# thu-pacman/chitu

Measured on AMD Instinct MI355X. Metric: output tok/s (bs=16) DeepSeek-R1 FP8 TP=8; HBM GB/s vs peak, higher is better.
Workload: dtype fp8_e4m3 weights+activations (W8A8, fp32 accumulate), bf16 attention

## Files before the change

chitu_amd/csrc/fp8_gemm.hip:

```cpp
#include "common.h"
#include "gemm_common.h"
#ifndef CHITU_GEMM_PHASE_MASK
#define CHITU_GEMM_PHASE_MASK 0
#endif

namespace chitu {

typedef long mfma_ab_t;

__device__ __forceinline__ mfma_ab_t pack_lo(const i32x4& v) {
    return (long)(((unsigned long long)(uint32_t)v[1] << 32) | (uint32_t)v[0]);
}
__device__ __forceinline__ mfma_ab_t pack_hi(const i32x4& v) {
    return (long)(((unsigned long long)(uint32_t)v[3] << 32) | (uint32_t)v[2]);
}

template <int MT>
struct GemmStage {
    W8Frag w;
    i32x4 x[MT][2];
    float xs[MT];
    float ws;
};

// ... 41 lines not shown
        const int off = kb << 7;
        if (!(dbg & 8)) {
            st.w.w[0] = __builtin_nontemporal_load(reinterpret_cast<const i32x4*>(wp0 + off));
            st.w.w[1] = __builtin_nontemporal_load(reinterpret_cast<const i32x4*>(wp1 + off));
        } else {
            st.w.w[0] = st.w.w[1] = i32x4{kb, lane, 3, 4};
        }
#pragma unroll
        for (int mt = 0; mt < MT; ++mt) {
            if (TM || (dbg & 16)) {
                st.x[mt][0] = *reinterpret_cast<const i32x4*>(xp[mt] + (size_t)kb * 2048);
                st.x[mt][1] = *reinterpret_cast<const i32x4*>(xp[mt] + (size_t)kb * 2048 + 1024);
            } else if (!(dbg & 1)) {
                st.x[mt][0] = *reinterpret_cast<const i32x4*>(xp[mt] + off);
                st.x[mt][1] = *reinterpret_cast<const i32x4*>(xp[mt] + off + 64);
            } else {
                st.x[mt][0] = st.x[mt][1] = i32x4{kb, lane, 1, 2};
            }
            st.xs[mt] = (dbg & 4) ? 1.0f : (TM || (dbg & 16)) ? xsp[mt][kb * 16] : xsp[mt][kb];
        }
        st.ws = wsp[kb];
    };
    auto compute = [&](const GemmStage<MT>& st) {
#pragma unroll
        for (int mt = 0; mt < MT; ++mt) {
            f32x4 blk;
            if (!(dbg & 2)) blk = w8a8_block_dot(st.w, st.x[mt][0], st.x[mt][1]);
            else
                blk = f32x4{__int_as_float(st.w.w[0][0] ^ st.x[mt][0][0]), __int_as_float(st.w.w[0][1] ^ st.x[mt][1][1]),
                            __int_as_float(st.w.w[1][2] ^ st.x[mt][0][2]), __int_as_float(st.w.w[1][3] ^ st.x[mt][1][3])};
#pragma unroll
            for (int r = 0; r < 4; ++r) acc[mt][r] += (blk[r] * st.xs[mt]) * st.ws;
        }
    };

    constexpr int D = DEEP ? 8 : MT >= 4 ? 2 : 4;
    GemmStage<MT> ring[D];
#pragma unroll
    for (int d = 0; d < D; ++d)
        if (kb0 + d < kb1) load(ring[d], kb0 + d);
    if (DEEP) CHITU_PROBE_MARK(1);
    for (int kb = kb0; kb < kb1; kb += D) {
#pragma unroll
        for (int d = 0; d < D; ++d) {
            if (kb + d < kb1) {
                compute(ring[d]);
                if (DEEP && kb == kb0 && d == 0) {
                    if (acc[0][0] == 1.2345e30f) CHITU_PROBE_MARK(9);
                    CHITU_PROBE_MARK(2);
                }
                if (kb + d + D < kb1) load(ring[d], kb + d + D);
            }
        }
    }
    if (DEEP) {
        if (acc[0][0] == 1.2345e30f) CHITU_PROBE_MARK(9);
        CHITU_PROBE_MARK(3);
    }

    gemm_epilogue_v2<MT, WK>(acc, red, out, out_dt, partial, M, N, S, m_base, n0);
    if (DEEP) CHITU_PROBE_MARK(4);
}

__global__ __launch_bounds__(256) void splitk_reduce_kernel(const float* __restrict__ partial,
                                                            void* __restrict__ out, int out_dt,
                                                            int S, int64_t MN) {
    for (int64_t i = ((int64_t)blockIdx.x * blockDim.x + threadIdx.x) * 4; i < MN;
         i += (int64_t)gridDim.x * blockDim.x * 4) {
        float v[4] = {0.f, 0.f, 0.f, 0.f};
        const int cnt = (int)min((int64_t)4, MN - i);
        for (int s = 0; s < S; ++s)
            for (int r = 0; r < cnt; ++r) v[r] += partial[(size_t)s * MN + i + r];
        for (int r = 0; r < cnt; ++r) {
            if (out_dt == 2) ((float*)out)[i + r] = v[r];
            else ((uint16_t*)out)[i + r] = out_dt == 0 ? f32_to_bf16(v[r]) : f32_to_f16(v[r]);
        }
    }
}

template <int MT, int WK>
__global__ __launch_bounds__(64 * WK) void soft_fp8_gemm_kernel(
    const bf16_t* __restrict__ X, const fp8_t* __restrict__ W, const float* __restrict__ WS,
    void* __restrict__ out, int out_dt, float* __restrict__ partial, int M, int N, int K, int S,
    int m_base) {
// ... 250 lines not shown
```

chitu_amd/csrc/gate.hip:

```cpp
#include "common.h"
#include "gemm_common.h"
#include "moe_align_device.h"

namespace chitu {

template <int MT>
struct Bf16Stage {
    s16x8 w[2];
    s16x8 x[MT][2];
};

template <int MT, int WK, bool DEEP = false>
__global__ __launch_bounds__(64 * WK) void bf16_gemm_kernel(const bf16_t* __restrict__ X,
                                                            const bf16_t* __restrict__ W,
                                                            void* __restrict__ out, int out_dt,
                                                            float* __restrict__ partial, int M, int N,
                                                            int K, int S, int m_base) {
    __shared__ float red[WK > 1 ? WK * MT * 256 : 1];
    const int lane = threadIdx.x & 63, wave = __builtin_amdgcn_readfirstlane(threadIdx.x >> 6);
    const int j = lane & 15, g = lane >> 4;
    const int n0 = blockIdx.x * 16;
    const int KB = K >> 6;
    const int T = S * WK;
    const int t = blockIdx.y * WK + wave;
    const int kb0 = (int)((long)KB * t / T), kb1 = (int)((long)KB * (t + 1) / T);
    const int eoff = ((j & 1) * 4 + g) * 8;
    const bf16_t* wp0 = W + (size_t)min(n0 + (j >> 1), N - 1) * K + eoff;
    const bf16_t* wp1 = W + (size_t)min(n0 + 8 + (j >> 1), N - 1) * K + eoff;
    const bf16_t* xp[MT];
#pragma unroll
    for (int mt = 0; mt < MT; ++mt) xp[mt] = X + (size_t)min(m_base + mt * 16 + j, M - 1) * K + g * 8;
    f32x4 e0[MT], o0[MT], e1[MT], o1[MT];
#pragma unroll
    for (int mt = 0; mt < MT; ++mt) e0[mt] = o0[mt] = e1[mt] = o1[mt] = f32x4{0.f, 0.f, 0.f, 0.f};
    auto load = [&](Bf16Stage<MT>& st, int kb) {
        const int off = kb << 6;
        st.w[0] = __builtin_nontemporal_load(reinterpret_cast<const s16x8*>(wp0 + off));
        st.w[1] = __builtin_nontemporal_load(reinterpret_cast<const s16x8*>(wp1 + off));
#pragma unroll
        for (int mt = 0; mt < MT; ++mt) {
            st.x[mt][0] = *reinterpret_cast<const s16x8*>(xp[mt] + off);
            st.x[mt][1] = *reinterpret_cast<const s16x8*>(xp[mt] + off + 32);
        }
    };
    auto compute = [&](const Bf16Stage<MT>& st) {
#pragma unroll
        for (int mt = 0; mt < MT; ++mt) {
            e0[mt] = __builtin_amdgcn_mfma_f32_16x16x32_bf16(st.w[0], st.x[mt][0], e0[mt], 0, 0, 0);
            o0[mt] = __builtin_amdgcn_mfma_f32_16x16x32_bf16(st.w[0], st.x[mt][1], o0[mt], 0, 0, 0);
            e1[mt] = __builtin_amdgcn_mfma_f32_16x16x32_bf16(st.w[1], st.x[mt][0], e1[mt], 0, 0, 0);
            o1[mt] = __builtin_amdgcn_mfma_f32_16x16x32_bf16(st.w[1], st.x[mt][1], o1[mt], 0, 0, 0);
        }
    };
    constexpr int D = DEEP ? 8 : MT >= 4 ? 2 : 4;
    Bf16Stage<MT> ring[D];
#pragma unroll
    for (int d = 0; d < D; ++d)
        if (kb0 + d < kb1) load(ring[d], kb0 + d);
    for (int kb = kb0; kb < kb1; kb += D) {
#pragma unroll
        for (int d = 0; d < D; ++d) {
            if (kb + d < kb1) {
                compute(ring[d]);
                if (kb + d + D < kb1) load(ring[d], kb + d + D);
            }
        }
    }
    f32x4 acc[MT];
#pragma unroll
    for (int mt = 0; mt < MT; ++mt)
        acc[mt] = f32x4{e0[mt][0] + o0[mt][1], e0[mt][2] + o0[mt][3], e1[mt][0] + o1[mt][1], e1[mt][2] + o1[mt][3]};
    gemm_epilogue_v2<MT, WK>(acc, red, out, out_dt, partial, M, N, S, m_base, n0);
}

template <int MT>
struct Bf16Stage2 {
    s16x8 wg[2], wu[2];
    s16x8 x[MT][2];
};

template <int MT, int WK>
__global__ __launch_bounds__(64 * WK) void bf16_gemm_silu_kernel(const bf16_t* __restrict__ X, const bf16_t* __restrict__ W,
                                                                 bf16_t* __restrict__ out, int M, int inter, int K,
                                                                 int m_base) {
    __shared__ float red[WK > 1 ? WK * MT * 512 : 1];
    const int lane = threadIdx.x & 63, wave = __builtin_amdgcn_readfirstlane(threadIdx.x >> 6);
    const int j = lane & 15, g = lane >> 4;
    const int n0 = blockIdx.x * 16;
    const int KB = K >> 6;
    const int kb0 = KB * wave / WK, kb1 = KB * (wave + 1) / WK;
    const int eoff = ((j & 1) * 4 + g) * 8;
    const int r0 = min(n0 + (j >> 1), inter - 1), r1 = min(n0 + 8 + (j >> 1), inter - 1);
    const bf16_t* gp0 = W + (size_t)r0 * K + eoff;
    const bf16_t* gp1 = W + (size_t)r1 * K + eoff;
    const bf16_t* up0 = W + (size_t)(inter + r0) * K + eoff;
    const bf16_t* up1 = W + (size_t)(inter + r1) * K + eoff;
    const bf16_t* xp[MT];
// ... 841 lines not shown
```

chitu_amd/csrc/gemm_common.h:

```cpp
#pragma once
#include "common.h"

namespace chitu {

template <int MT, int WK>
__device__ __forceinline__ void gemm_epilogue(f32x4 (&acc)[MT], float* red, void* out, int out_dt,
                                              float* partial, int M, int N, int S, int m_base,
                                              int n0) {
    const int lane = threadIdx.x & 63;
    const int wave = __builtin_amdgcn_readfirstlane(threadIdx.x >> 6);
    const int j = lane & 15, g = lane >> 4;
    auto store = [&](int mt, const f32x4& v) {
        const int m = m_base + mt * 16 + j;
        const int n = n0 + g * 4;
        if (m >= M) return;
        if (S > 1) {
            float* dst = partial + ((size_t)blockIdx.y * M + m) * N + n;
            if (n + 3 < N && (N & 3) == 0) *reinterpret_cast<f32x4*>(dst) = v;
            else
                for (int r = 0; r < 4 && n + r < N; ++r) dst[r] = v[r];
        } else if (out_dt == 2) {
            float* dst = (float*)out + (size_t)m * N + n;
            for (int r = 0; r < 4 && n + r < N; ++r) dst[r] = v[r];
        } else {
// ... 56 lines not shown
#else
    f32x4 d = __builtin_amdgcn_mfma_f32_16x16x32_fp8_fp8(frag_lo(a0), frag_lo(b0), z, 0, 0, 0);
    d = __builtin_amdgcn_mfma_f32_16x16x32_fp8_fp8(frag_hi(a0), frag_hi(b0), d, 0, 0, 0);
    d = __builtin_amdgcn_mfma_f32_16x16x32_fp8_fp8(frag_lo(a1), frag_lo(b1), d, 0, 0, 0);
    return __builtin_amdgcn_mfma_f32_16x16x32_fp8_fp8(frag_hi(a1), frag_hi(b1), d, 0, 0, 0);
#endif
}

__device__ __forceinline__ void fold_scaled(f32x4& acc, const f32x4& d, float a_s, float b_s) {
    const f32x4 t = d * a_s;
    acc = __builtin_elementwise_fma(t, f32x4{b_s, b_s, b_s, b_s}, acc);
}

__device__ __forceinline__ void w8_lane_ptrs(const fp8_t* Wbase, int n0, int n_rows, int K, int j, int g,
                                             const fp8_t*& p0, const fp8_t*& p1) {
    const int off = ((j & 1) * 4 + g) * 16;
    p0 = Wbase + (size_t)min(n0 + (j >> 1), n_rows - 1) * K + off;
    p1 = Wbase + (size_t)min(n0 + 8 + (j >> 1), n_rows - 1) * K + off;
}

__device__ __forceinline__ f32x4 w8a8_block_dot(const W8Frag& f, const i32x4& x0, const i32x4& x1) {
    const f32x4 z = f32x4{0.f, 0.f, 0.f, 0.f};
    f32x4 e0 = __builtin_amdgcn_mfma_f32_16x16x32_fp8_fp8(frag_lo(f.w[0]), frag_lo(x0), z, 0, 0, 0);
    f32x4 o0 = __builtin_amdgcn_mfma_f32_16x16x32_fp8_fp8(frag_lo(f.w[0]), frag_lo(x1), z, 0, 0, 0);
    f32x4 e1 = __builtin_amdgcn_mfma_f32_16x16x32_fp8_fp8(frag_lo(f.w[1]), frag_lo(x0), z, 0, 0, 0);
    f32x4 o1 = __builtin_amdgcn_mfma_f32_16x16x32_fp8_fp8(frag_lo(f.w[1]), frag_lo(x1), z, 0, 0, 0);
    e0 = __builtin_amdgcn_mfma_f32_16x16x32_fp8_fp8(frag_hi(f.w[0]), frag_hi(x0), e0, 0, 0, 0);
    o0 = __builtin_amdgcn_mfma_f32_16x16x32_fp8_fp8(frag_hi(f.w[0]), frag_hi(x1), o0, 0, 0, 0);
    e1 = __builtin_amdgcn_mfma_f32_16x16x32_fp8_fp8(frag_hi(f.w[1]), frag_hi(x0), e1, 0, 0, 0);
    o1 = __builtin_amdgcn_mfma_f32_16x16x32_fp8_fp8(frag_hi(f.w[1]), frag_hi(x1), o1, 0, 0, 0);
    return f32x4{e0[0] + o0[1], e0[2] + o0[3], e1[0] + o1[1], e1[2] + o1[3]};
}

__device__ __forceinline__ int w8_out_col(int n0, int g, int e) { return n0 + (e >> 1) * 8 + 2 * g + (e & 1); }

template <int MT, int WK>
__device__ __forceinline__ void gemm_epilogue_v2(f32x4 (&acc)[MT], float* red, void* out, int out_dt,
                                                 float* partial, int M, int N, int S, int m_base, int n0) {
    const int lane = threadIdx.x & 63;
    const int wave = __builtin_amdgcn_readfirstlane(threadIdx.x >> 6);
    const int j = lane & 15, g = lane >> 4;
    auto store = [&](int mt, const f32x4& v) {
        const int m = m_base + mt * 16 + j;
        if (m >= M) return;
#pragma unroll
        for (int h = 0; h < 2; ++h) {
            const int n = n0 + h * 8 + 2 * g;
            const float a = v[2 * h], b = v[2 * h + 1];
            if (S > 1) {
                float* dst = partial + ((size_t)blockIdx.y * M + m) * N + n;
                if (n < N) dst[0] = a;
                if (n + 1 < N) dst[1] = b;
            } else if (out_dt == 2) {
                float* dst = (float*)out + (size_t)m * N + n;
                if (n < N) dst[0] = a;
                if (n + 1 < N) dst[1] = b;
            } else {
                uint16_t* dst = (uint16_t*)out + (size_t)m * N + n;
                const uint16_t ha = out_dt == 0 ? f32_to_bf16(a) : f32_to_f16(a);
                const uint16_t hb = out_dt == 0 ? f32_to_bf16(b) : f32_to_f16(b);
                if (n + 1 < N && (N & 1) == 0) *reinterpret_cast<uint32_t*>(dst) = (uint32_t)ha | ((uint32_t)hb << 16);
                else {
                    if (n < N) dst[0] = ha;
                    if (n + 1 < N) dst[1] = hb;
                }
            }
// ... 66 lines not shown
```

chitu_amd/csrc/moe.hip:

```cpp
#include "common.h"
#include "gemm_common.h"
#ifndef CHITU_MOE_PROBE_MASK
#define CHITU_MOE_PROBE_MASK 0
#endif

namespace chitu {

struct MoeStage {
    W8Frag w;
    i32x4 x[2];
    float xs, ws;
};

__device__ __forceinline__ void moe_store_tile(bf16_t* out_row, int n0, int g, int N, const f32x4& acc, float rw) {
#pragma unroll
    for (int h = 0; h < 2; ++h) {
        const int n = n0 + h * 8 + 2 * g;
        const uint16_t a = f32_to_bf16(acc[2 * h] * rw), b = f32_to_bf16(acc[2 * h + 1] * rw);
        if (n + 1 < N && (N & 1) == 0) *reinterpret_cast<uint32_t*>(out_row + n) = (uint32_t)a | ((uint32_t)b << 16);
        else {
            if (n < N) out_row[n] = a;
            if (n + 1 < N) out_row[n + 1] = b;
        }
    }
}

__device__ __forceinline__ float moe_routed_weight(const void* topk_w, int w_dt, int slot) {
    if (w_dt == 0) return bf16_to_f32(((const bf16_t*)topk_w)[slot]);
    if (w_dt == 1) return f16_to_f32(((const uint16_t*)topk_w)[slot]);
    return ((const float*)topk_w)[slot];
}

template <int WK, int NW, int D>
__global__ __launch_bounds__(64 * WK * NW) void moe_gemm1_kernel(
    const fp8_t* __restrict__ Xq, const float* __restrict__ Xs, const fp8_t* __restrict__ W,
    const float* __restrict__ Ws, const int32_t* __restrict__ sorted_ids,
    const int32_t* __restrict__ expert_ids, const int32_t* __restrict__ num_post_pad,
    bf16_t* __restrict__ out, int numel, int topk, int N, int K) {
    static_assert(WK == 1 || NW == 1, "either split K or tile N inside a workgroup");
    __shared__ float red[WK > 1 ? WK * 256 : 1];
    const int mb = blockIdx.y;
    if (mb * 16 >= *num_post_pad) return;
    const int lane = threadIdx.x & 63, wave = __builtin_amdgcn_readfirstlane(threadIdx.x >> 6);
    const int j = lane & 15, g = lane >> 4;
    const int n0 = (NW > 1 ? blockIdx.x * NW + wave : blockIdx.x) * 16;
    if (NW > 1 && n0 >= N) return;
    const int KB = K >> 7;
    const int slot = sorted_ids[mb * 16 + j];
    const bool valid = slot < numel;
    const int e = expert_ids[mb];
    f32x4 acc = f32x4{0.f, 0.f, 0.f, 0.f};
    if (e >= 0) {
        const int kw = NW > 1 ? 0 : wave;
        const int kb0 = KB * kw / WK, kb1 = KB * (kw + 1) / WK;
        const int slot0 = __builtin_amdgcn_readfirstlane(slot);
        const int token = (valid ? slot : min(slot0, numel - 1)) / topk;
        const fp8_t* xp = Xq + (size_t)token * K + g * 16;
        const float* xsp = Xs + (size_t)token * KB;
        const fp8_t *wp0, *wp1;
        w8_lane_ptrs(W + (size_t)e * N * K, n0, N, K, j, g, wp0, wp1);
        const float* wsp = Ws + ((size_t)e * ((N + 127) >> 7) + (n0 >> 7)) * KB;
        auto load = [&](MoeStage& st, int kb) {
            const int off = kb << 7;
            st.w.w[0] = __builtin_nontemporal_load(reinterpret_cast<const i32x4*>(wp0 + off));
            st.w.w[1] = __builtin_nontemporal_load(reinterpret_cast<const i32x4*>(wp1 + off));
            st.x[0] = *reinterpret_cast<const i32x4*>(xp + off);
            st.x[1] = *reinterpret_cast<const i32x4*>(xp + off + 64);
            st.xs = xsp[kb];
            st.ws = wsp[kb];
        };
        auto compute = [&](const MoeStage& st) {
            const f32x4 blk = w8a8_block_dot(st.w, st.x[0], st.x[1]);
#pragma unroll
            for (int r = 0; r < 4; ++r) acc[r] += (blk[r] * st.xs) * st.ws;
        };
        MoeStage ring[D];
#pragma unroll
        for (int d = 0; d < D; ++d)
            if (kb0 + d < kb1) load(ring[d], kb0 + d);
        for (int kb = kb0; kb < kb1; kb += D) {
#pragma unroll
            for (int d = 0; d < D; ++d) {
                if (kb + d < kb1) {
                    compute(ring[d]);
                    if (kb + d + D < kb1) load(ring[d], kb + d + D);
                }
            }
        }
    }
    if (WK > 1) {
        *reinterpret_cast<f32x4*>(&red[(wave * 64 + lane) * 4]) = acc;
        __syncthreads();
        if (wave != 0) return;
        acc = f32x4{0.f, 0.f, 0.f, 0.f};
#pragma unroll
        for (int w = 0; w < WK; ++w) {
            const f32x4 v = *reinterpret_cast<const f32x4*>(&red[(w * 64 + lane) * 4]);
#pragma unroll
            for (int r = 0; r < 4; ++r) acc[r] += v[r];
        }
    }
    if (!valid) return;
    moe_store_tile(out + (size_t)slot * N, n0, g, N, acc, 1.0f);
}

struct MoeStage2 {
    W8Frag wg, wu;
    i32x4 x[2];
    float xs, wsg, wsu;
};

template <int WK, int D, bool Q = false>
__global__ __launch_bounds__(Q ? 512 : 64 * WK) void moe_gemm1_silu_kernel(
    const fp8_t* __restrict__ Xq, const float* __restrict__ Xs, const fp8_t* __restrict__ W,
    const float* __restrict__ Ws, const int32_t* __restrict__ sorted_ids,
    const int32_t* __restrict__ expert_ids, const int32_t* __restrict__ num_post_pad,
    bf16_t* __restrict__ out, int numel, int topk, int I, int K, fp8_t* __restrict__ hq = nullptr,
    float* __restrict__ hs = nullptr, float eps = 0.f) {
    static_assert(!Q || WK == 1, "the quantising epilogue owns whole K");
    __shared__ float red[WK > 1 ? WK * 512 : 1];
    __shared__ float qmax[Q ? 8 * 16 : 1];
    const int mb = blockIdx.y;
    if (mb * 16 >= *num_post_pad) return;
    const int lane = threadIdx.x & 63;
    const int wave_id = __builtin_amdgcn_readfirstlane(threadIdx.x >> 6);
    const int wave = Q ? 0 : wave_id;
    const int j = lane & 15, g = lane >> 4;
    const int n0 = (Q ? blockIdx.x * 8 + wave_id : blockIdx.x) * 16;
    const int N = 2 * I;
    const int KB = K >> 7;
    const int slot = sorted_ids[mb * 16 + j];
    const bool valid = slot < numel;
    const int e = expert_ids[mb];
    f32x4 ag = f32x4{0.f, 0.f, 0.f, 0.f}, au = f32x4{0.f, 0.f, 0.f, 0.f};
    if (e >= 0) {
        const int kb0 = KB * wave / WK, kb1 = KB * (wave + 1) / WK;
        const int slot0 = __builtin_amdgcn_readfirstlane(slot);
        const int token = (valid ? slot : min(slot0, numel - 1)) / topk;
        const fp8_t* xp = Xq + (size_t)token * K + g * 16;
        const float* xsp = Xs + (size_t)token * KB;
        if (CHITU_MOE_PROBE_MASK & 1) {
            xp = Xq + (size_t)(g * 16 + (token & 15)) * 16;
            xsp = Xs + (token & 15);
        }
        const fp8_t* Wb = W + (size_t)e * N * K;
        const fp8_t *gp0, *gp1, *up0, *up1;
        w8_lane_ptrs(Wb, n0, N, K, j, g, gp0, gp1);
        w8_lane_ptrs(Wb, I + n0, N, K, j, g, up0, up1);
        const float* wsb = Ws + (size_t)e * ((N + 127) >> 7) * KB;
        const float* wsgp = wsb + (size_t)(n0 >> 7) * KB;
        const float* wsup = wsb + (size_t)((I + n0) >> 7) * KB;
        auto load = [&](MoeStage2& st, int kb) {
            const int off = kb << 7;
            st.wg.w[0] = __builtin_nontemporal_load(reinterpret_cast<const i32x4*>(gp0 + off));
            st.wg.w[1] = __builtin_nontemporal_load(reinterpret_cast<const i32x4*>(gp1 + off));
            st.wu.w[0] = __builtin_nontemporal_load(reinterpret_cast<const i32x4*>(up0 + off));
            st.wu.w[1] = __builtin_nontemporal_load(reinterpret_cast<const i32x4*>(up1 + off));
            if (CHITU_MOE_PROBE_MASK & 1) {
                st.x[0] = *reinterpret_cast<const i32x4*>(xp + (size_t)kb * 2048);
                st.x[1] = *reinterpret_cast<const i32x4*>(xp + (size_t)kb * 2048 + 1024);
                st.xs = xsp[kb * 16];
            } else {
                st.x[0] = *reinterpret_cast<const i32x4*>(xp + off);
                st.x[1] = *reinterpret_cast<const i32x4*>(xp + off + 64);
                st.xs = xsp[kb];
            }
            st.wsg = wsgp[kb];
            st.wsu = wsup[kb];
        };
        auto compute = [&](const MoeStage2& st) {
            const f32x4 bg = w8a8_block_dot(st.wg, st.x[0], st.x[1]);
            const f32x4 bu = w8a8_block_dot(st.wu, st.x[0], st.x[1]);
#pragma unroll
            for (int r = 0; r < 4; ++r) {
                ag[r] += (bg[r] * st.xs) * st.wsg;
                au[r] += (bu[r] * st.xs) * st.wsu;
            }
        };
        MoeStage2 ring[D];
#pragma unroll
        for (int d = 0; d < D; ++d)
            if (kb0 + d < kb1) load(ring[d], kb0 + d);
        for (int kb = kb0; kb < kb1; kb += D) {
#pragma unroll
            for (int d = 0; d < D; ++d) {
                if (kb + d < kb1) {
                    compute(ring[d]);
                    if (kb + d + D < kb1) load(ring[d], kb + d + D);
                }
            }
        }
    }
    if (WK > 1) {
        *reinterpret_cast<f32x4*>(&red[(wave * 128 + lane) * 4]) = ag;
        *reinterpret_cast<f32x4*>(&red[(wave * 128 + 64 + lane) * 4]) = au;
        __syncthreads();
        if (wave != 0) return;
        ag = f32x4{0.f, 0.f, 0.f, 0.f};
        au = f32x4{0.f, 0.f, 0.f, 0.f};
#pragma unroll
        for (int w = 0; w < WK; ++w) {
            const f32x4 vg = *reinterpret_cast<const f32x4*>(&red[(w * 128 + lane) * 4]);
            const f32x4 vu = *reinterpret_cast<const f32x4*>(&red[(w * 128 + 64 + lane) * 4]);
#pragma unroll
            for (int r = 0; r < 4; ++r) {
                ag[r] += vg[r];
                au[r] += vu[r];
            }
        }
    }
    if (!Q && !valid) return;
    f32x4 h;
#pragma unroll
    for (int r = 0; r < 4; ++r) {
        const float gv = round_bf16(ag[r]), uv = round_bf16(au[r]);
        const float sl = round_bf16(gv / (1.0f + expf(-gv)));
        h[r] = round_bf16(sl * uv);
    }
    if (!Q) {
        moe_store_tile(out + (size_t)slot * I, n0, g, I, h, 1.0f);
        return;
    }
    float amax = __builtin_fmaxf(__builtin_fmaxf(__builtin_fabsf(h[0]), __builtin_fabsf(h[1])),
                                 __builtin_fmaxf(__builtin_fabsf(h[2]), __builtin_fabsf(h[3])));
// ... 98 lines not shown
        }
    }
#pragma unroll
    for (int t = 0; t < NT; ++t) {
        const int n0 = (tile0 + t) * 16;
        if (n0 >= N) break;
        f32x4 acc = f32x4{0.f, 0.f, 0.f, 0.f};
        if (e >= 0) {
            const float* wsp = Ws + ((size_t)e * ((N + 127) >> 7) + (n0 >> 7)) * KB;
#pragma unroll
            for (int kb = 0; kb < KBMAX; ++kb) {
                if (kb < KB) {
                    const f32x4 blk = w8a8_block_dot(wf[t][kb], x[kb][0], x[kb][1]);
                    const float ws = wsp[kb];
#pragma unroll
                    for (int r = 0; r < 4; ++r) acc[r] += (blk[r] * xs[kb]) * ws;
                }
            }
        }
        if (valid) moe_store_tile(out + (size_t)slot * N, n0, g, N, acc, rw);
    }
}

template <int KB, int NT, int ROUNDS>
__global__ __launch_bounds__(256) void moe_gemm2_q_kernel(
    const bf16_t* __restrict__ Hb, const fp8_t* __restrict__ W, const float* __restrict__ Ws,
    const int32_t* __restrict__ sorted_ids, const int32_t* __restrict__ expert_ids,
    const int32_t* __restrict__ num_post_pad, const void* __restrict__ topk_w, int w_dt,
    bf16_t* __restrict__ out, int numel, int N, int mul_weight, float eps) {
    constexpr int I = KB * 128;
    constexpr int HPW = (2 * KB + 3) / 4;
    __shared__ float amax_lds[2 * KB][16];
    __shared__ i32x4 xq_lds[2 * KB][64];
    const int mb = blockIdx.y;
    if (mb * 16 >= *num_post_pad) return;
    const int lane = threadIdx.x & 63, wave = __builtin_amdgcn_readfirstlane(threadIdx.x >> 6);
    const int j = lane & 15, g = lane >> 4;
    const int slot = sorted_ids[mb * 16 + j];
    const bool valid = slot < numel;
    const int e = expert_ids[mb];
    auto tile_of = [&](int r) { return ((blockIdx.x * ROUNDS + r) * 4 + wave) * NT; };
    if (e < 0) {
#pragma unroll
        for (int r = 0; r < ROUNDS; ++r)
#pragma unroll
            for (int t = 0; t < NT; ++t) {
                const int n0 = (tile_of(r) + t) * 16;
                if (n0 < N && valid) moe_store_tile(out + (size_t)slot * N, n0, g, N, f32x4{0.f, 0.f, 0.f, 0.f}, 1.0f);
            }
        return;
    }
    const int row = valid ? slot : 0;
    const bf16_t* hrow = Hb + (size_t)row * I;
    i32x4 hraw[HPW][2];
#pragma unroll
    for (int q = 0; q < HPW; ++q) {
        const int hb = min(wave + 4 * q, 2 * KB - 1);
        hraw[q][0] = *reinterpret_cast<const i32x4*>(hrow + hb * 64 + g * 16);
        hraw[q][1] = *reinterpret_cast<const i32x4*>(hrow + hb * 64 + g * 16 + 8);
    }
    const int last_tile = (N - 1) >> 4;
    const fp8_t* We = W + (size_t)e * N * I;
    W8Frag wf[ROUNDS > 1 ? 2 : 1][NT][KB];
    auto load_round = [&](W8Frag (&dst)[NT][KB], int r) {
#pragma unroll
        for (int t = 0; t < NT; ++t) {
            const int n0 = min(tile_of(r) + t, last_tile) * 16;
            const fp8_t *wp0, *wp1;
            w8_lane_ptrs(We, n0, N, I, j, g, wp0, wp1);
#pragma unroll
            for (int kb = 0; kb < KB; ++kb) {
                dst[t][kb].w[0] = __builtin_nontemporal_load(reinterpret_cast<const i32x4*>(wp0 + (kb << 7)));
                dst[t][kb].w[1] = __builtin_nontemporal_load(reinterpret_cast<const i32x4*>(wp1 + (kb << 7)));
            }
        }
    };
    load_round(wf[0], 0);
    const float rw = (mul_weight && valid) ? moe_routed_weight(topk_w, w_dt, slot) : 1.0f;
    float h[HPW][16];
#pragma unroll
    for (int q = 0; q < HPW; ++q) {
        const int hb = wave + 4 * q;
        float amax = 0.f;
#pragma unroll
        for (int i = 0; i < 16; ++i) {
            const uint32_t u = (uint32_t)hraw[q][i >> 3][(i >> 1) & 3];
            h[q][i] = (i & 1) ? __uint_as_float(u & 0xffff0000u) : __uint_as_float(u << 16);
            amax = __builtin_fmaxf(amax, __builtin_fabsf(h[q][i]));
        }
        amax = __builtin_fmaxf(amax, __shfl_xor(amax, 16, 64));
        amax = __builtin_fmaxf(amax, __shfl_xor(amax, 32, 64));
        if (g == 0 && hb < 2 * KB) amax_lds[hb][j] = amax;
    }
    __syncthreads();
#pragma unroll
    for (int q = 0; q < HPW; ++q) {
        const int hb = wave + 4 * q;
        if (hb < 2 * KB) {
            const float sc = __builtin_fmaxf(__builtin_fmaxf(amax_lds[hb & ~1][j], amax_lds[hb | 1][j]), eps) / 448.0f;
            float lo[8], hi[8];
#pragma unroll
            for (int i = 0; i < 8; ++i) {
                lo[i] = h[q][i];
                hi[i] = h[q][8 + i];
            }
            const i32x2 a = quant8_fp8<true>(lo, sc), b = quant8_fp8<true>(hi, sc);
            xq_lds[hb][lane] = i32x4{a[0], a[1], b[0], b[1]};
        }
    }
    __syncthreads();
    i32x4 x[KB][2];
    float xs[KB];
#pragma unroll
    for (int kb = 0; kb < KB; ++kb) {
        x[kb][0] = xq_lds[2 * kb][lane];
        x[kb][1] = xq_lds[2 * kb + 1][lane];
        xs[kb] = __builtin_fmaxf(__builtin_fmaxf(amax_lds[2 * kb][j], amax_lds[2 * kb + 1][j]), eps) / 448.0f;
    }
    const float* wse = Ws + (size_t)e * ((N + 127) >> 7) * KB;
#pragma unroll
    for (int r = 0; r < ROUNDS; ++r) {
        if (r + 1 < ROUNDS) load_round(wf[(r + 1) & 1], r + 1);
#pragma unroll
        for (int t = 0; t < NT; ++t) {
            const int n0 = (tile_of(r) + t) * 16;
            f32x4 acc = f32x4{0.f, 0.f, 0.f, 0.f};
            const float* wsp = wse + (size_t)(min(n0, N - 1) >> 7) * KB;
#pragma unroll
            for (int kb = 0; kb < KB; ++kb) {
                const f32x4 blk = w8a8_block_dot(wf[r & 1][t][kb], x[kb][0], x[kb][1]);
                const float ws = wsp[kb];
#pragma unroll
                for (int rr = 0; rr < 4; ++rr) acc[rr] += (blk[rr] * xs[kb]) * ws;
            }
            if (valid && n0 < N) moe_store_tile(out + (size_t)slot * N, n0, g, N, acc, rw);
        }
    }
}

template <int WK>
__global__ __launch_bounds__(64 * WK) void moe_gemm2_generic_kernel(
    const fp8_t* __restrict__ Hq, const float* __restrict__ Hs, const fp8_t* __restrict__ W,
    const float* __restrict__ Ws, const int32_t* __restrict__ sorted_ids,
    const int32_t* __restrict__ expert_ids, const int32_t* __restrict__ num_post_pad,
    const void* __restrict__ topk_w, int w_dt, bf16_t* __restrict__ out, int numel, int N, int I,
    int mul_weight) {
    __shared__ float red[WK > 1 ? WK * 256 : 1];
    const int mb = blockIdx.y;
    if (mb * 16 >= *num_post_pad) return;
    const int lane = threadIdx.x & 63, wave = __builtin_amdgcn_readfirstlane(threadIdx.x >> 6);
    const int j = lane & 15, g = lane >> 4;
    const int n0 = blockIdx.x * 16;
// ... 179 lines not shown
        }
#undef LAUNCHG
    }
    CHITU_RETURN_LAUNCH_STATUS();
}

extern "C" int chitu_hip_moe_gemm1_silu_fp8(const void* a_fp8, const float* a_scale, const void* w1_fp8,
                                            const float* w1_scale, const int32_t* sorted_token_ids,
                                            const int32_t* expert_ids, const int32_t* num_tokens_post_pad,
                                            void* h_bf16, int64_t numel, int32_t topk, int64_t inter_size,
                                            int64_t K, int64_t max_mblocks, void* stream) {
    using namespace chitu;
    CHITU_REQUIRE(a_fp8 && a_scale && w1_fp8 && w1_scale && sorted_token_ids && expert_ids);
    CHITU_REQUIRE(num_tokens_post_pad && h_bf16);
    CHITU_REQUIRE(numel >= 0 && topk >= 1 && inter_size >= 16 && K >= 128 && max_mblocks >= 0);
    if (K % 128 != 0 || inter_size % 16 != 0) return CHITU_ERR_UNSUPPORTED;
    if (numel == 0 || max_mblocks == 0) return CHITU_OK;
    const int n_tiles = (int)(inter_size / 16);
    const int64_t wgs = 2 * (int64_t)n_tiles * (numel < max_mblocks ? numel : max_mblocks);
    const int KB = (int)(K / 128);
    int WK = wgs <= 640 ? 8 : wgs <= 1536 ? 4 : wgs <= 3200 ? 2 : 1;
    debug_override(kOptMoeGemm1WK, WK);
    while (WK > 1 && WK > KB) WK >>= 1;
    int D = WK >= 4 ? 2 : 3;
    debug_override(kOptMoeGemm1D, D);
    hipStream_t st = (hipStream_t)stream;
    const dim3 grid((unsigned)n_tiles, (unsigned)max_mblocks);
#define LAUNCH1S(WKV, DV)                                                                                     \
    hipLaunchKernelGGL((moe_gemm1_silu_kernel<WKV, DV>), grid, dim3(64 * WKV), 0, st, (const fp8_t*)a_fp8, a_scale, \
                       (const fp8_t*)w1_fp8, w1_scale, sorted_token_ids, expert_ids, num_tokens_post_pad,      \
                       (bf16_t*)h_bf16, (int)numel, (int)topk, (int)inter_size, (int)K)
    if (WK == 8) { if (D == 2) LAUNCH1S(8, 2); else if (D == 3) LAUNCH1S(8, 3); else LAUNCH1S(8, 4); }
    else if (WK == 4) { if (D == 2) LAUNCH1S(4, 2); else if (D == 3) LAUNCH1S(4, 3); else LAUNCH1S(4, 4); }
    else if (WK == 2) { if (D == 4) LAUNCH1S(2, 4); else LAUNCH1S(2, 3); }
    else { if (D == 4) LAUNCH1S(1, 4); else LAUNCH1S(1, 3); }
#undef LAUNCH1S
    CHITU_RETURN_LAUNCH_STATUS();
}

extern "C" int chitu_hip_moe_gemm2_quant_fp8(const void* h_bf16, const void* w2_fp8, const float* w2_scale,
                                             const int32_t* sorted_token_ids, const int32_t* expert_ids,
                                             const int32_t* num_tokens_post_pad, const void* topk_weights,
                                             int weights_dtype, int32_t mul_routed_weight, void* out_bf16,
                                             int64_t numel, int64_t N, int64_t inter_size, int64_t max_mblocks,
                                             float eps, void* stream) {
    using namespace chitu;
    CHITU_REQUIRE(h_bf16 && w2_fp8 && w2_scale && sorted_token_ids && expert_ids);
    CHITU_REQUIRE(num_tokens_post_pad && out_bf16 && (topk_weights || !mul_routed_weight));
    CHITU_REQUIRE(numel >= 0 && N >= 1 && inter_size >= 128 && max_mblocks >= 0);
    CHITU_REQUIRE(weights_dtype >= 0 && weights_dtype <= 2);
    if (inter_size % 128 != 0 || inter_size > 512) return CHITU_ERR_UNSUPPORTED;
    if (numel == 0 || max_mblocks == 0) return CHITU_OK;
    hipStream_t st = (hipStream_t)stream;
    const int n_tiles = (int)((N + 15) / 16);
    const int KB = (int)(inter_size / 128);
    const int64_t mbs = numel < max_mblocks ? numel : max_mblocks;
#define LAUNCH2Q(KBV, NTV, RV)                                                                       \
    hipLaunchKernelGGL((moe_gemm2_q_kernel<KBV, NTV, RV>),                                           \
                       dim3((unsigned)((n_tiles + 4 * NTV * RV - 1) / (4 * NTV * RV)), (unsigned)max_mblocks), \
                       dim3(256), 0, st, (const bf16_t*)h_bf16, (const fp8_t*)w2_fp8, w2_scale,      \
                       sorted_token_ids, expert_ids, num_tokens_post_pad, topk_weights, weights_dtype, \
                       (bf16_t*)out_bf16, (int)numel, (int)N, (int)mul_routed_weight, eps)
    const bool many = (int64_t)n_tiles * mbs > 50000;
    int cfg = many ? 24 : 21;
    debug_override(kOptMoeGemm2Cfg, cfg);
    switch (KB) {
        case 1: LAUNCH2Q(1, 2, 1); break;
        case 2:
// ... 28 lines not shown
```

chitu_amd/fused_moe.py:

```python

import os
from typing import List, Optional, Tuple

import torch

from . import _lib, workspace
from ._lib import check, f32, float_dtype_code, i32, i64, int_dtype_code, ptr, require_cuda, stream_ptr

__all__ = [
    "moe_align_block_size",
    "per_token_group_quant_fp8",
    "fused_experts",
    "fused_experts_impl",
]


def ceil_div(a, b):
    return (a + b - 1) // b


def cuda_moe_align_block_size(
    topk_ids: torch.Tensor,
    num_experts: int,
    block_size: int,
# ... 12 lines not shown
    if cumsum_buffer.numel() < num_experts + 1:
        raise RuntimeError("cumsum_buffer too small")
    check(
        _lib.lib().chitu_hip_moe_align_block_size(
            ptr(topk_ids), int_dtype_code(topk_ids.dtype), i64(topk_ids.numel()), i32(num_experts),
            i32(block_size), ptr(sorted_token_ids), i64(sorted_token_ids.numel()), ptr(experts_ids),
            i64(experts_ids.numel()), ptr(num_tokens_post_pad), ptr(cumsum_buffer), i32(0), stream_ptr(),
        ),
        "cuda_moe_align_block_size",
    )


def _expert_map_i32(expert_map: Optional[torch.Tensor], num_experts: int, dev) -> Optional[torch.Tensor]:
    if expert_map is None:
        return None
    assert expert_map.numel() >= num_experts, "expert_map must cover every global expert id"
    if expert_map.dtype != torch.int32 or expert_map.device != dev or not expert_map.is_contiguous():
        expert_map = expert_map.to(device=dev, dtype=torch.int32).contiguous()
    return expert_map


def moe_align_block_size(
    topk_ids: torch.Tensor,
    block_size: int,
    num_experts: int,
    expert_map: torch.Tensor = None,
) -> Tuple[torch.Tensor, torch.Tensor, torch.Tensor]:
    require_cuda(topk_ids)
    if not topk_ids.is_contiguous():
        topk_ids = topk_ids.contiguous()
    numel = topk_ids.numel()
    max_num_tokens_padded = numel + num_experts * (block_size - 1)
    dev = topk_ids.device
    sorted_ids = torch.empty((max_num_tokens_padded,), dtype=torch.int32, device=dev)
    max_num_m_blocks = ceil_div(max_num_tokens_padded, block_size)
    expert_ids = torch.empty((max_num_m_blocks,), dtype=torch.int32, device=dev)
    num_tokens_post_pad = torch.empty((1), dtype=torch.int32, device=dev)
    cumsum_buffer = torch.empty((num_experts + 1,), dtype=torch.int32, device=dev)
    emap = _expert_map_i32(expert_map, num_experts, dev)
    check(
        _lib.lib().chitu_hip_moe_align_block_size_mapped(
            ptr(topk_ids), int_dtype_code(topk_ids.dtype), i64(numel), i32(num_experts), i32(block_size),
            ptr(sorted_ids), i64(sorted_ids.numel()), ptr(expert_ids), i64(expert_ids.numel()),
            ptr(num_tokens_post_pad), ptr(cumsum_buffer), i32(1), ptr(emap), stream_ptr(),
        ),
        "moe_align_block_size",
    )
    return sorted_ids, expert_ids, num_tokens_post_pad


def per_token_group_quant_fp8(
    x: torch.Tensor,
    group_size: int,
    eps: float = 1e-10,
    dtype: Optional[torch.dtype] = None,
    column_major_scales: bool = False,
) -> Tuple[torch.Tensor, torch.Tensor]:
    if dtype is None:
        dtype = torch.float8_e4m3fn
    assert dtype == torch.float8_e4m3fn, "only torch.float8_e4m3fn (OCP) is supported"
    assert x.shape[-1] % group_size == 0, (
        f"the last dimension of `x` {x.shape[-1]} must be divisible " f"by `group_size` {group_size}"
    )
    assert x.stride(-1) == 1, "`x` groups must be contiguous"
    assert not column_major_scales, "column-major scales are not used on this path"
    require_cuda(x)
    if not x.is_contiguous():
        x = x.contiguous()
# ... 128 lines not shown
    numel = num_tokens * topk
    if not topk_ids.is_contiguous():
        topk_ids = topk_ids.contiguous()
    if not topk_weights.is_contiguous():
        topk_weights = topk_weights.contiguous()

    def rnd(n):
        return (n + 255) // 256 * 256

    tiled = (_MOE_TILED_MIN_TOKENS > 0 and num_tokens >= _MOE_TILED_MIN_TOKENS and aligned is None and I % 128 == 0
             and Nout % 8 == 0 and numel >= _MOE_TILED_MIN_PER_EXPERT * global_num_experts)
    block_m = _MOE_TILED_BLOCK_M if tiled else _MOE_BLOCK_M
    cap = numel + global_num_experts * (block_m - 1)
    nblk = ceil_div(cap, block_m)
    KB = K // 128
    sizes = [
        ("sorted", cap * 4), ("experts", nblk * 4), ("npost", 4), ("cumsum", (global_num_experts + 1) * 4),
        ("a1q", num_tokens * K), ("a1s", num_tokens * KB * 4), ("c1", numel * N * 2),
        ("a2q", numel * I), ("a2s", numel * (I // 128) * 4), ("c3", numel * Nout * 2),
    ]
    total = sum(rnd(n) for _, n in sizes)
    ws = workspace.get(total, dev, "moe")
    base = ws.data_ptr()
    off = {}
    cur = 0
    for name, n in sizes:
        off[name] = base + cur
        cur += rnd(n)
    import ctypes as _ct

    P = lambda name: _ct.c_void_p(off[name])
    lib = _lib.lib()
    st = stream_ptr()
    max_mblocks = min(nblk, numel)

    if aligned is None:
        emap = _expert_map_i32(expert_map, global_num_experts, dev)
        check(
            lib.chitu_hip_moe_align_block_size_mapped(
                ptr(topk_ids), int_dtype_code(topk_ids.dtype), i64(numel), i32(global_num_experts),
                i32(block_m), P("sorted"), i64(cap), P("experts"), i64(nblk), P("npost"), P("cumsum"),
                i32(1), ptr(emap), st,
            ),
            "moe_align_block_size",
        )
        sorted_p, experts_ptr, npost_p = P("sorted"), P("experts"), P("npost")
    else:
        a_sorted, a_experts, a_npost = aligned
        require_cuda(a_sorted, a_experts, a_npost)
        assert a_sorted.dtype == torch.int32 and a_experts.dtype == torch.int32 and a_npost.dtype == torch.int32
        assert a_sorted.numel() == cap and a_experts.numel() == nblk, "aligned buffers must come from block 16 over global_num_experts"
        sorted_p, experts_ptr, npost_p = ptr(a_sorted), ptr(a_experts), ptr(a_npost)
    if a1_quant is None:
        check(
            lib.chitu_hip_act_quant_fp8(
                ptr(hidden_states), float_dtype_code(hidden_states.dtype), i64(num_tokens), i64(K), i32(128),
                i32(1), f32(1e-10), P("a1q"), P("a1s"), st,
            ),
            "moe quant1",
        )
        a1q_p, a1s_p = P("a1q"), P("a1s")
    else:
        aq, as_ = a1_quant
        assert aq.is_contiguous() and as_.is_contiguous() and aq.numel() == num_tokens * K
        assert as_.dtype == torch.float32 and as_.numel() == num_tokens * KB
        a1q_p, a1s_p = ptr(aq), ptr(as_)
    if tiled:
# ... 221 lines not shown
```

Baseline: 205.9.

## Issue weight loads before routing-dependent activation loads in GEMM and MoE rings

Adds a shared ring_run helper that pipelines the K loop. It issues the weight prefetches first, then computes token and activation addresses, then the activation loads, with sched_barrier fences and asm barriers to pin the order. The MoE kernels now read num_post_pad, expert id and slot together before the early exit, so weight streaming can start while the routing-dependent address chain resolves. The routed-weight load is hoisted early, and it adds D=2 launch variants, padded sorted_ids allocation and a capped max_mblocks. Trade-offs are extra scheduling constraints, more code paths, and possible register pressure from the asm pins.

```diff
diff --git a/chitu_amd/csrc/fp8_gemm.hip b/chitu_amd/csrc/fp8_gemm.hip
--- a/chitu_amd/csrc/fp8_gemm.hip
+++ b/chitu_amd/csrc/fp8_gemm.hip
@@ -97,24 +97,34 @@
 #pragma unroll
             for (int r = 0; r < 4; ++r) acc[mt][r] += (blk[r] * st.xs[mt]) * st.ws;
         }
+        if (!DEEP) {
+#pragma unroll
+            for (int mt = 0; mt < MT; ++mt) asm("" : "+v"(acc[mt]));
+        }
     };
 
     constexpr int D = DEEP ? 8 : MT >= 4 ? 2 : 4;
     GemmStage<MT> ring[D];
-#pragma unroll
-    for (int d = 0; d < D; ++d)
-        if (kb0 + d < kb1) load(ring[d], kb0 + d);
-    if (DEEP) CHITU_PROBE_MARK(1);
-    for (int kb = kb0; kb < kb1; kb += D) {
-#pragma unroll
-        for (int d = 0; d < D; ++d) {
-            if (kb + d < kb1) {
-                compute(ring[d]);
-                if (DEEP && kb == kb0 && d == 0) {
-                    if (acc[0][0] == 1.2345e30f) CHITU_PROBE_MARK(9);
-                    CHITU_PROBE_MARK(2);
+    if (!DEEP) {
+        auto none = [] {};
+        auto no_load = [](GemmStage<MT>&, int) {};
+        ring_run<D>(kb0, kb1, ring, load, no_load, none, compute);
+    } else {
+#pragma unroll
+        for (int d = 0; d < D; ++d)
+            if (kb0 + d < kb1) load(ring[d], kb0 + d);
+        CHITU_PROBE_MARK(1);
+        for (int kb = kb0; kb < kb1; kb += D) {
+#pragma unroll
+            for (int d = 0; d < D; ++d) {
+                if (kb + d < kb1) {
+                    compute(ring[d]);
+                    if (kb == kb0 && d == 0) {
+                        if (acc[0][0] == 1.2345e30f) CHITU_PROBE_MARK(9);
+                        CHITU_PROBE_MARK(2);
+                    }
+                    if (kb + d + D < kb1) load(ring[d], kb + d + D);
                 }
-                if (kb + d + D < kb1) load(ring[d], kb + d + D);
             }
         }
     }
diff --git a/chitu_amd/csrc/gate.hip b/chitu_amd/csrc/gate.hip
--- a/chitu_amd/csrc/gate.hip
+++ b/chitu_amd/csrc/gate.hip
@@ -54,15 +54,21 @@
     };
     constexpr int D = DEEP ? 8 : MT >= 4 ? 2 : 4;
     Bf16Stage<MT> ring[D];
-#pragma unroll
-    for (int d = 0; d < D; ++d)
-        if (kb0 + d < kb1) load(ring[d], kb0 + d);
-    for (int kb = kb0; kb < kb1; kb += D) {
-#pragma unroll
-        for (int d = 0; d < D; ++d) {
-            if (kb + d < kb1) {
-                compute(ring[d]);
-                if (kb + d + D < kb1) load(ring[d], kb + d + D);
+    if (!DEEP) {
+        auto none = [] {};
+        auto no_load = [](Bf16Stage<MT>&, int) {};
+        ring_run<D>(kb0, kb1, ring, load, no_load, none, compute);
+    } else {
+#pragma unroll
+        for (int d = 0; d < D; ++d)
+            if (kb0 + d < kb1) load(ring[d], kb0 + d);
+        for (int kb = kb0; kb < kb1; kb += D) {
+#pragma unroll
+            for (int d = 0; d < D; ++d) {
+                if (kb + d < kb1) {
+                    compute(ring[d]);
+                    if (kb + d + D < kb1) load(ring[d], kb + d + D);
+                }
             }
         }
     }
diff --git a/chitu_amd/csrc/gemm_common.h b/chitu_amd/csrc/gemm_common.h
--- a/chitu_amd/csrc/gemm_common.h
+++ b/chitu_amd/csrc/gemm_common.h
@@ -112,6 +112,67 @@
     return f32x4{e0[0] + o0[1], e0[2] + o0[3], e1[0] + o1[1], e1[2] + o1[3]};
 }
 
+template <int D, class Stage, class LoadW, class LoadX, class Addr, class Compute>
+__device__ __forceinline__ void ring_run(int kb0, int kb1, Stage (&ring)[D], const LoadW& load_w, const LoadX& load_x,
+                                         const Addr& addr, const Compute& compute) {
+    int kb = kb0;
+    auto round = [&]() {
+#pragma unroll
+        for (int d = 0; d < D; ++d) {
+            compute(ring[d]);
+            __builtin_amdgcn_sched_barrier(0);
+            load_w(ring[d], kb + d + D);
+            load_x(ring[d], kb + d + D);
+            __builtin_amdgcn_sched_barrier(0);
+        }
+        kb += D;
+    };
+    if (kb0 + 2 * D <= kb1) {
+#pragma unroll
+        for (int d = 0; d < D; ++d) load_w(ring[d], kb0 + d);
+        __builtin_amdgcn_sched_barrier(0);
+        addr();
+#pragma unroll
+        for (int d = 0; d < D; ++d) load_x(ring[d], kb0 + d);
+        __builtin_amdgcn_sched_barrier(0);
+        round();
+        while (kb + 2 * D <= kb1) round();
+#pragma unroll
+        for (int d = 0; d < D; ++d) {
+            compute(ring[d]);
+            __builtin_amdgcn_sched_barrier(0);
+            if (kb + d + D < kb1) {
+                load_w(ring[d], kb + d + D);
+                load_x(ring[d], kb + d + D);
+            }
+        }
+    } else {
+#pragma unroll
+        for (int d = 0; d < D; ++d)
+            if (kb0 + d < kb1) load_w(ring[d], kb0 + d);
+        __builtin_amdgcn_sched_barrier(0);
+        addr();
+#pragma unroll
+        for (int d = 0; d < D; ++d)
+            if (kb0 + d < kb1) load_x(ring[d], kb0 + d);
+        __builtin_amdgcn_sched_barrier(0);
+#pragma unroll
+        for (int d = 0; d < D; ++d) {
+            if (kb + d < kb1) {
+                compute(ring[d]);
+                if (kb + d + D < kb1) {
+                    load_w(ring[d], kb + d + D);
+                    load_x(ring[d], kb + d + D);
+                }
+            }
+        }
+    }
+    kb += D;
+#pragma unroll
+    for (int d = 0; d < D; ++d)
+        if (kb + d < kb1) compute(ring[d]);
+}
+
 __device__ __forceinline__ int w8_out_col(int n0, int g, int e) { return n0 + (e >> 1) * 8 + 2 * g + (e & 1); }
 
 template <int MT, int WK>
diff --git a/chitu_amd/csrc/moe.hip b/chitu_amd/csrc/moe.hip
--- a/chitu_amd/csrc/moe.hip
+++ b/chitu_amd/csrc/moe.hip
@@ -29,6 +29,14 @@
     if (w_dt == 0) return bf16_to_f32(((const bf16_t*)topk_w)[slot]);
     if (w_dt == 1) return f16_to_f32(((const uint16_t*)topk_w)[slot]);
     return ((const float*)topk_w)[slot];
+}
+
+__device__ __forceinline__ void moe_plan(const int32_t* __restrict__ sorted_ids, const int32_t* __restrict__ expert_ids,
+                                         const int32_t* __restrict__ num_post_pad, int mb, int j, int& npp, int& e, int& slot) {
+    npp = *num_post_pad;
+    e = expert_ids[mb];
+    slot = sorted_ids[mb * 16 + j];
+    asm("" : "+s"(npp), "+s"(e), "+v"(slot));
 }
 
 template <int WK, int NW, int D>
@@ -39,31 +47,33 @@
     bf16_t* __restrict__ out, int numel, int topk, int N, int K) {
     static_assert(WK == 1 || NW == 1, "either split K or tile N inside a workgroup");
     __shared__ float red[WK > 1 ? WK * 256 : 1];
-    const int mb = blockIdx.y;
-    if (mb * 16 >= *num_post_pad) return;
+    int mb = blockIdx.y;
+    asm("" : "+s"(mb) : "s"(Xq), "s"(Xs), "s"(W), "s"(Ws), "s"(sorted_ids), "s"(expert_ids), "s"(num_post_pad), "s"(out), "s"(numel),
+        "s"(topk), "s"(N), "s"(K));
     const int lane = threadIdx.x & 63, wave = __builtin_amdgcn_readfirstlane(threadIdx.x >> 6);
     const int j = lane & 15, g = lane >> 4;
+    int npp, e, slot;
+    moe_plan(sorted_ids, expert_ids, num_post_pad, mb, j, npp, e, slot);
+    if (mb * 16 >= npp) return;
     const int n0 = (NW > 1 ? blockIdx.x * NW + wave : blockIdx.x) * 16;
     if (NW > 1 && n0 >= N) return;
     const int KB = K >> 7;
-    const int slot = sorted_ids[mb * 16 + j];
     const bool valid = slot < numel;
-    const int e = expert_ids[mb];
     f32x4 acc = f32x4{0.f, 0.f, 0.f, 0.f};
     if (e >= 0) {
         const int kw = NW > 1 ? 0 : wave;
         const int kb0 = KB * kw / WK, kb1 = KB * (kw + 1) / WK;
-        const int slot0 = __builtin_amdgcn_readfirstlane(slot);
-        const int token = (valid ? slot : min(slot0, numel - 1)) / topk;
-        const fp8_t* xp = Xq + (size_t)token * K + g * 16;
-        const float* xsp = Xs + (size_t)token * KB;
         const fp8_t *wp0, *wp1;
         w8_lane_ptrs(W + (size_t)e * N * K, n0, N, K, j, g, wp0, wp1);
-        const float* wsp = Ws + ((size_t)e * ((N + 127) >> 7) + (n0 >> 7)) * KB;
-        auto load = [&](MoeStage& st, int kb) {
+        const fp8_t* xp;
+        const float *xsp, *wsp;
+        auto load_w = [&](MoeStage& st, int kb) {
             const int off = kb << 7;
             st.w.w[0] = __builtin_nontemporal_load(reinterpret_cast<const i32x4*>(wp0 + off));
             st.w.w[1] = __builtin_nontemporal_load(reinterpret_cast<const i32x4*>(wp1 + off));
+        };
+        auto load_x = [&](MoeStage& st, int kb) {
+            const int off = kb << 7;
             st.x[0] = *reinterpret_cast<const i32x4*>(xp + off);
             st.x[1] = *reinterpret_cast<const i32x4*>(xp + off + 64);
             st.xs = xsp[kb];
@@ -73,20 +83,17 @@
             const f32x4 blk = w8a8_block_dot(st.w, st.x[0], st.x[1]);
 #pragma unroll
             for (int r = 0; r < 4; ++r) acc[r] += (blk[r] * st.xs) * st.ws;
+            asm("" : "+v"(acc));
+        };
+        auto addr = [&]() {
+            const int slot0 = __builtin_amdgcn_readfirstlane(slot);
+            const int token = (valid ? slot : min(slot0, numel - 1)) / topk;
+            xp = Xq + (size_t)token * K + g * 16;
+            xsp = Xs + (size_t)token * KB;
+            wsp = Ws + ((size_t)e * ((N + 127) >> 7) + (n0 >> 7)) * KB;
         };
         MoeStage ring[D];
-#pragma unroll
-        for (int d = 0; d < D; ++d)
-            if (kb0 + d < kb1) load(ring[d], kb0 + d);
-        for (int kb = kb0; kb < kb1; kb += D) {
-#pragma unroll
-            for (int d = 0; d < D; ++d) {
-                if (kb + d < kb1) {
-                    compute(ring[d]);
-                    if (kb + d + D < kb1) load(ring[d], kb + d + D);
-                }
-            }
-        }
+        ring_run<D>(kb0, kb1, ring, load_w, load_x, addr, compute);
     }
     if (WK > 1) {
         *reinterpret_cast<f32x4*>(&red[(wave * 64 + lane) * 4]) = acc;
@@ -120,42 +127,38 @@
     static_assert(!Q || WK == 1, "the quantising epilogue owns whole K");
     __shared__ float red[WK > 1 ? WK * 512 : 1];
     __shared__ float qmax[Q ? 8 * 16 : 1];
-    const int mb = blockIdx.y;
-    if (mb * 16 >= *num_post_pad) return;
+    int mb = blockIdx.y;
+    asm("" : "+s"(mb) : "s"(Xq), "s"(Xs), "s"(W), "s"(Ws), "s"(sorted_ids), "s"(expert_ids), "s"(num_post_pad), "s"(out), "s"(numel),
+        "s"(topk), "s"(I), "s"(K));
     const int lane = threadIdx.x & 63;
     const int wave_id = __builtin_amdgcn_readfirstlane(threadIdx.x >> 6);
     const int wave = Q ? 0 : wave_id;
     const int j = lane & 15, g = lane >> 4;
+    int npp, e, slot;
+    moe_plan(sorted_ids, expert_ids, num_post_pad, mb, j, npp, e, slot);
+    if (mb * 16 >= npp) return;
     const int n0 = (Q ? blockIdx.x * 8 + wave_id : blockIdx.x) * 16;
     const int N = 2 * I;
     const int KB = K >> 7;
-    const int slot = sorted_ids[mb * 16 + j];
     const bool valid = slot < numel;
-    const int e = expert_ids[mb];
     f32x4 ag = f32x4{0.f, 0.f, 0.f, 0.f}, au = f32x4{0.f, 0.f, 0.f, 0.f};
     if (e >= 0) {
         const int kb0 = KB * wave / WK, kb1 = KB * (wave + 1) / WK;
-        const int slot0 = __builtin_amdgcn_readfirstlane(slot);
-        const int token = (valid ? slot : min(slot0, numel - 1)) / topk;
-        const fp8_t* xp = Xq + (size_t)token * K + g * 16;
-        const float* xsp = Xs + (size_t)token * KB;
-        if (CHITU_MOE_PROBE_MASK & 1) {
-            xp = Xq + (size_t)(g * 16 + (token & 15)) * 16;
-            xsp = Xs + (token & 15);
-        }
         const fp8_t* Wb = W + (size_t)e * N * K;
         const fp8_t *gp0, *gp1, *up0, *up1;
         w8_lane_ptrs(Wb, n0, N, K, j, g, gp0, gp1);
         w8_lane_ptrs(Wb, I + n0, N, K, j, g, up0, up1);
-        const float* wsb = Ws + (size_t)e * ((N + 127) >> 7) * KB;
-        const float* wsgp = wsb + (size_t)(n0 >> 7) * KB;
-        const float* wsup = wsb + (size_t)((I + n0) >> 7) * KB;
-        auto load = [&](MoeStage2& st, int kb) {
+        const fp8_t* xp;
+        const float *xsp, *wsgp, *wsup;
+        auto load_w = [&](MoeStage2& st, int kb) {
             const int off = kb << 7;
             st.wg.w[0] = __builtin_nontemporal_load(reinterpret_cast<const i32x4*>(gp0 + off));
             st.wg.w[1] = __builtin_nontemporal_load(reinterpret_cast<const i32x4*>(gp1 + off));
             st.wu.w[0] = __builtin_nontemporal_load(reinterpret_cast<const i32x4*>(up0 + off));
             st.wu.w[1] = __builtin_nontemporal_load(reinterpret_cast<const i32x4*>(up1 + off));
+        };
+        auto load_x = [&](MoeStage2& st, int kb) {
+            const int off = kb << 7;
             if (CHITU_MOE_PROBE_MASK & 1) {
                 st.x[0] = *reinterpret_cast<const i32x4*>(xp + (size_t)kb * 2048);
                 st.x[1] = *reinterpret_cast<const i32x4*>(xp + (size_t)kb * 2048 + 1024);
@@ -176,20 +179,23 @@
                 ag[r] += (bg[r] * st.xs) * st.wsg;
                 au[r] += (bu[r] * st.xs) * st.wsu;
             }
+            asm("" : "+v"(ag), "+v"(au));
+        };
+        auto addr = [&]() {
+            const int slot0 = __builtin_amdgcn_readfirstlane(slot);
+            const int token = (valid ? slot : min(slot0, numel - 1)) / topk;
+            xp = Xq + (size_t)token * K + g * 16;
+            xsp = Xs + (size_t)token * KB;
+            if (CHITU_MOE_PROBE_MASK & 1) {
+                xp = Xq + (size_t)(g * 16 + (token & 15)) * 16;
+                xsp = Xs + (token & 15);
+            }
+            const float* wsb = Ws + (size_t)e * ((N + 127) >> 7) * KB;
+            wsgp = wsb + (size_t)(n0 >> 7) * KB;
+            wsup = wsb + (size_t)((I + n0) >> 7) * KB;
         };
         MoeStage2 ring[D];
-#pragma unroll
-        for (int d = 0; d < D; ++d)
-            if (kb0 + d < kb1) load(ring[d], kb0 + d);
-        for (int kb = kb0; kb < kb1; kb += D) {
-#pragma unroll
-            for (int d = 0; d < D; ++d) {
-                if (kb + d < kb1) {
-                    compute(ring[d]);
-                    if (kb + d + D < kb1) load(ring[d], kb + d + D);
-                }
-            }
-        }
+        ring_run<D>(kb0, kb1, ring, load_w, load_x, addr, compute);
     }
     if (WK > 1) {
         *reinterpret_cast<f32x4*>(&red[(wave * 128 + lane) * 4]) = ag;
@@ -354,13 +360,15 @@
     constexpr int HPW = (2 * KB + 3) / 4;
     __shared__ float amax_lds[2 * KB][16];
     __shared__ i32x4 xq_lds[2 * KB][64];
-    const int mb = blockIdx.y;
-    if (mb * 16 >= *num_post_pad) return;
+    int mb = blockIdx.y;
+    asm("" : "+s"(mb) : "s"(Hb), "s"(W), "s"(Ws), "s"(sorted_ids), "s"(expert_ids), "s"(num_post_pad), "s"(topk_w), "s"(w_dt), "s"(out),
+        "s"(numel), "s"(N), "s"(mul_weight), "s"(eps));
     const int lane = threadIdx.x & 63, wave = __builtin_amdgcn_readfirstlane(threadIdx.x >> 6);
     const int j = lane & 15, g = lane >> 4;
-    const int slot = sorted_ids[mb * 16 + j];
+    int npp, e, slot;
+    moe_plan(sorted_ids, expert_ids, num_post_pad, mb, j, npp, e, slot);
+    if (mb * 16 >= npp) return;
     const bool valid = slot < numel;
-    const int e = expert_ids[mb];
     auto tile_of = [&](int r) { return ((blockIdx.x * ROUNDS + r) * 4 + wave) * NT; };
     if (e < 0) {
 #pragma unroll
@@ -372,6 +380,8 @@
             }
         return;
     }
+    uint32_t rw_bits = 0;
+    if (mul_weight && valid) rw_bits = w_dt == 2 ? ((const uint32_t*)topk_w)[slot] : (uint32_t)((const uint16_t*)topk_w)[slot];
     const int row = valid ? slot : 0;
     const bf16_t* hrow = Hb + (size_t)row * I;
     i32x4 hraw[HPW][2];
@@ -398,7 +408,6 @@
         }
     };
     load_round(wf[0], 0);
-    const float rw = (mul_weight && valid) ? moe_routed_weight(topk_w, w_dt, slot) : 1.0f;
     float h[HPW][16];
 #pragma unroll
     for (int q = 0; q < HPW; ++q) {
@@ -440,6 +449,10 @@
         xs[kb] = __builtin_fmaxf(__builtin_fmaxf(amax_lds[2 * kb][j], amax_lds[2 * kb + 1][j]), eps) / 448.0f;
     }
     const float* wse = Ws + (size_t)e * ((N + 127) >> 7) * KB;
+    const float rw = !(mul_weight && valid) ? 1.0f
+                     : w_dt == 0            ? bf16_to_f32((bf16_t)rw_bits)
+                     : w_dt == 1            ? f16_to_f32((uint16_t)rw_bits)
+                                            : __uint_as_float(rw_bits);
 #pragma unroll
     for (int r = 0; r < ROUNDS; ++r) {
         if (r + 1 < ROUNDS) load_round(wf[(r + 1) & 1], r + 1);
@@ -685,8 +698,8 @@
                        (bf16_t*)h_bf16, (int)numel, (int)topk, (int)inter_size, (int)K)
     if (WK == 8) { if (D == 2) LAUNCH1S(8, 2); else if (D == 3) LAUNCH1S(8, 3); else LAUNCH1S(8, 4); }
     else if (WK == 4) { if (D == 2) LAUNCH1S(4, 2); else if (D == 3) LAUNCH1S(4, 3); else LAUNCH1S(4, 4); }
-    else if (WK == 2) { if (D == 4) LAUNCH1S(2, 4); else LAUNCH1S(2, 3); }
-    else { if (D == 4) LAUNCH1S(1, 4); else LAUNCH1S(1, 3); }
+    else if (WK == 2) { if (D == 2) LAUNCH1S(2, 2); else if (D == 4) LAUNCH1S(2, 4); else LAUNCH1S(2, 3); }
+    else { if (D == 2) LAUNCH1S(1, 2); else if (D == 4) LAUNCH1S(1, 4); else LAUNCH1S(1, 3); }
 #undef LAUNCH1S
     CHITU_RETURN_LAUNCH_STATUS();
 }
diff --git a/chitu_amd/fused_moe.py b/chitu_amd/fused_moe.py
--- a/chitu_amd/fused_moe.py
+++ b/chitu_amd/fused_moe.py
@@ -68,8 +68,8 @@
     numel = topk_ids.numel()
     max_num_tokens_padded = numel + num_experts * (block_size - 1)
     dev = topk_ids.device
-    sorted_ids = torch.empty((max_num_tokens_padded,), dtype=torch.int32, device=dev)
     max_num_m_blocks = ceil_div(max_num_tokens_padded, block_size)
+    sorted_ids = torch.empty((max_num_m_blocks * block_size,), dtype=torch.int32, device=dev)[:max_num_tokens_padded]
     expert_ids = torch.empty((max_num_m_blocks,), dtype=torch.int32, device=dev)
     num_tokens_post_pad = torch.empty((1), dtype=torch.int32, device=dev)
     cumsum_buffer = torch.empty((num_experts + 1,), dtype=torch.int32, device=dev)
@@ -264,7 +264,7 @@
     P = lambda name: _ct.c_void_p(off[name])
     lib = _lib.lib()
     st = stream_ptr()
-    max_mblocks = min(nblk, numel)
+    max_mblocks = min(nblk, numel, cap // block_m)
 
     if aligned is None:
         emap = _expert_map_i32(expert_map, global_num_experts, dev)
```

New measurement: 206.6, median of 6. About the same (+0.3%).
